# taithenguyen/ppls

Measured on AMD Instinct MI355X. Metric: accepted subintervals/sec + FP64 F-evals/sec at 1/2/4/8 MI355X, EPSILON=1e-10, higher is better.
Workload: dtype f64

## Files before the change

ppls_amd/csrc/aq_device.h:

```cpp
#pragma once
#include <hip/hip_runtime.h>
#include <stdint.h>

#include <type_traits>

#include "aquad.h"
#include "aq_libm.h"

#pragma clang fp contract(off)

namespace aq {

enum : unsigned { ERRB_TIMEOUT = 1, ERRB_OVERFLOW = 2, ERRB_DEPTH = 4 };

__device__ __forceinline__ unsigned cu_slot() {
    const unsigned hw = __builtin_amdgcn_s_getreg((31 << 11) | 4);
    const unsigned xcc = __builtin_amdgcn_s_getreg((3 << 11) | 20);
    const unsigned cu = (hw >> 8) & 15u, sh = (hw >> 12) & 1u, se = (hw >> 13) & 7u;
    return ((xcc & 7u) << 8) | (((se << 1) | sh) << 4) | cu;
}

__device__ __forceinline__ double wave_sum(double v) {
#pragma unroll
    for (int o = 32; o > 0; o >>= 1) v += __shfl_xor(v, o, 64);
// ... 121 lines not shown
            s[k].refine = fabs(s[k].area2 - lr2e[k]) > eps2;
            if constexpr (step_has_diff<S>) s[k].diff = s[k].area2 - lr2e[k];
        } else {
            const double lrarea = lr2e[k] / 2;
            const double larea = (fl[k] + fmid[k]) * wl[k] / 2;
            const double rarea = (fmid[k] + fr[k]) * wr[k] / 2;
            s[k].area2 = larea + rarea;
            s[k].refine = fabs((larea + rarea) - lrarea) > eps2;
            if constexpr (step_has_diff<S>) s[k].diff = (larea + rarea) - lrarea;
        }
    }
}

struct Step2c {
    double fmid, l2, r2, area2;
    bool refine;
};
template <int FID>
__device__ __forceinline__ void pair_step_carry(double ha, double hb, double fa, double fm, double fb, double lr0,
                                                double lr1, double eps2, const ExpEntry* __restrict__ tab,
                                                Step2c (&s)[2], double& m, double& hm, const ExpConsts& kk,
                                                int range_hint, unsigned long long out_mask) {
    static_assert(doubled_areas<FID>(), "carried areas are doubled areas");
    m = ha + hb;
    hm = 0.5 * m;
    const double mid[2] = {ha + hm, hm + hb};
    const double fl[2] = {fa, fm}, fr[2] = {fm, fb}, lr[2] = {lr0, lr1};
    double wl[2], wr[2];
    wl[0] = __fma_rn(ha, -2.0, mid[0]);
    wl[1] = mid[1] - m;
    wr[0] = m - mid[0];
    wr[1] = __fma_rn(hb, 2.0, -mid[1]);
#pragma unroll
    for (int k = 0; k < 2; ++k) asm volatile("" : "+v"(wl[k]), "+v"(wr[k]));
    double fmid[2];
    integrand_k<FID, 2, (f_scale<FID>() != 1.0)>(mid, fmid, tab, kk, range_hint, out_mask);
#pragma unroll
    for (int k = 0; k < 2; ++k) {
        s[k].fmid = fmid[k];
        s[k].l2 = (fl[k] + fmid[k]) * wl[k];
        s[k].r2 = (fmid[k] + fr[k]) * wr[k];
        s[k].area2 = s[k].l2 + s[k].r2;
        s[k].refine = fabs(s[k].area2 - lr[k]) > eps2;
    }
}

__host__ __device__ __forceinline__ void two_sum(double a, double b, double& s, double& e) {
    s = a + b;
    const double bb = s - a;
    e = (a - (s - bb)) + (b - bb);
}
__host__ __device__ __forceinline__ void dd_add(double& hi, double& lo, double v) {
    double s, e;
    two_sum(hi, v, s, e);
    hi = s;
    lo += e;
}
__host__ __device__ __forceinline__ void dd_add_dd(double& hi, double& lo, double h2, double l2) {
    double s, e;
    two_sum(hi, h2, s, e);
    e += lo + l2;
    two_sum(s, e, hi, lo);
}
__device__ __forceinline__ void masked_add(double& acc, double v, unsigned long long mask) {
    unsigned long long saved;
    asm("s_and_saveexec_b64 %1, %3\n\t"
        "v_add_f64 %0, %0, %2\n\t"
        "s_mov_b64 exec, %1"
        : "+v"(acc), "=&s"(saved)
        : "v"(v), "s"(mask)
        : "scc");
}

__device__ __forceinline__ void masked_max(unsigned& m, unsigned v, unsigned long long mask) {
    unsigned long long saved;
    asm("s_and_saveexec_b64 %1, %3\n\t"
        "v_max_u32 %0, %0, %2\n\t"
        "s_mov_b64 exec, %1"
        : "+v"(m), "=&s"(saved)
        : "v"(v), "s"(mask)
        : "scc");
}

__device__ __forceinline__ void masked_acc3(double& hi, double a0, unsigned long long l0m, double a1,
                                            unsigned long long l1m, unsigned& m, unsigned v, unsigned long long am) {
    unsigned long long saved;
    asm("s_mov_b64 %1, exec\n\t"
        "s_mov_b64 exec, %5\n\t"
        "v_add_f64 %0, %0, %3\n\t"
        "s_mov_b64 exec, %6\n\t"
        "v_add_f64 %0, %0, %4\n\t"
        "s_mov_b64 exec, %7\n\t"
        "v_max_u32_sdwa %2, %2, %8 dst_sel:DWORD dst_unused:UNUSED_PAD src0_sel:DWORD src1_sel:BYTE_0\n\t"
        "s_mov_b64 exec, %1"
        : "+v"(hi), "=&s"(saved), "+v"(m)
        : "v"(a0), "v"(a1), "s"(l0m), "s"(l1m), "s"(am), "v"(v));
}

__device__ __forceinline__ void masked_err4(double& sg, double& ab, double d0, unsigned long long l0m, double d1,
                                            unsigned long long l1m) {
    unsigned long long saved;
    asm("s_mov_b64 %2, exec\n\t"
        "s_mov_b64 exec, %5\n\t"
        "v_add_f64 %0, %0, %3\n\t"
        "v_add_f64 %1, %1, |%3|\n\t"
        "s_mov_b64 exec, %6\n\t"
        "v_add_f64 %0, %0, %4\n\t"
        "v_add_f64 %1, %1, |%4|\n\t"
        "s_mov_b64 exec, %2"
        : "+v"(sg), "+v"(ab), "=&s"(saved)
        : "v"(d0), "v"(d1), "s"(l0m), "s"(l1m));
}

__device__ __forceinline__ void wave_sum_dd(double& hi, double& lo) {
#pragma unroll
    for (int o = 32; o > 0; o >>= 1) {
        const double h2 = __shfl_xor(hi, o, 64), l2 = __shfl_xor(lo, o, 64);
        dd_add_dd(hi, lo, h2, l2);
    }
}

enum : int { DPP_XOR1 = 0xB1, DPP_XOR2 = 0x4E, DPP_HALF_MIRROR = 0x141, DPP_MIRROR = 0x140 };
template <int CTRL>
__device__ __forceinline__ unsigned dpp_u(unsigned v) {
    return (unsigned)__builtin_amdgcn_update_dpp(0, (int)v, CTRL, 0xF, 0xF, false);
}
template <int CTRL>
__device__ __forceinline__ double dpp_d(double v) {
    const unsigned long long b = (unsigned long long)__double_as_longlong(v);
    const unsigned lo = dpp_u<CTRL>((unsigned)b), hi = dpp_u<CTRL>((unsigned)(b >> 32));
    return __longlong_as_double((long long)(((unsigned long long)hi << 32) | lo));
}
__device__ __forceinline__ double readlane_d(double v, int l) {
    const unsigned long long b = (unsigned long long)__double_as_longlong(v);
    const unsigned lo = __builtin_amdgcn_readlane((unsigned)b, l), hi = __builtin_amdgcn_readlane((unsigned)(b >> 32), l);
    return __longlong_as_double((long long)(((unsigned long long)hi << 32) | lo));
}
template <typename Op>
__device__ __forceinline__ unsigned wave_reduce_u(unsigned v, Op op) {
    v = op(v, dpp_u<DPP_XOR1>(v));
    v = op(v, dpp_u<DPP_XOR2>(v));
    v = op(v, dpp_u<DPP_HALF_MIRROR>(v));
    v = op(v, dpp_u<DPP_MIRROR>(v));
    return op(op(__builtin_amdgcn_readlane(v, 0), __builtin_amdgcn_readlane(v, 16)),
              op(__builtin_amdgcn_readlane(v, 32), __builtin_amdgcn_readlane(v, 48)));
}
__device__ __forceinline__ unsigned wave_add_full(unsigned v) {
    return wave_reduce_u(v, [](unsigned x, unsigned y) { return x + y; });
}
__device__ __forceinline__ unsigned wave_max_full(unsigned v) {
    return wave_reduce_u(v, [](unsigned x, unsigned y) { return x > y ? x : y; });
}
__device__ __forceinline__ unsigned wave_or_full(unsigned v) {
    return wave_reduce_u(v, [](unsigned x, unsigned y) { return x | y; });
}
__device__ __forceinline__ double wave_sum_d_full(double v) {
    v += dpp_d<DPP_XOR1>(v);
    v += dpp_d<DPP_XOR2>(v);
    v += dpp_d<DPP_HALF_MIRROR>(v);
    v += dpp_d<DPP_MIRROR>(v);
    return (readlane_d(v, 0) + readlane_d(v, 16)) + (readlane_d(v, 32) + readlane_d(v, 48));
}
__device__ __forceinline__ void row_sum_dd(double& hi, double& lo) {
    double h2 = dpp_d<DPP_XOR1>(hi), l2 = dpp_d<DPP_XOR1>(lo);
    dd_add_dd(hi, lo, h2, l2);
    h2 = dpp_d<DPP_XOR2>(hi); l2 = dpp_d<DPP_XOR2>(lo);
    dd_add_dd(hi, lo, h2, l2);
    h2 = dpp_d<DPP_HALF_MIRROR>(hi); l2 = dpp_d<DPP_HALF_MIRROR>(lo);
    dd_add_dd(hi, lo, h2, l2);
    h2 = dpp_d<DPP_MIRROR>(hi); l2 = dpp_d<DPP_MIRROR>(lo);
    dd_add_dd(hi, lo, h2, l2);
}
__device__ __forceinline__ void wave_sum_dd_full(double& hi, double& lo) {
    double h2 = dpp_d<DPP_XOR1>(hi), l2 = dpp_d<DPP_XOR1>(lo);
    dd_add_dd(hi, lo, h2, l2);
    h2 = dpp_d<DPP_XOR2>(hi); l2 = dpp_d<DPP_XOR2>(lo);
    dd_add_dd(hi, lo, h2, l2);
    h2 = dpp_d<DPP_HALF_MIRROR>(hi); l2 = dpp_d<DPP_HALF_MIRROR>(lo);
    dd_add_dd(hi, lo, h2, l2);
    h2 = dpp_d<DPP_MIRROR>(hi); l2 = dpp_d<DPP_MIRROR>(lo);
    dd_add_dd(hi, lo, h2, l2);
    double h0 = readlane_d(hi, 0), l0 = readlane_d(lo, 0), h1 = readlane_d(hi, 16), l1 = readlane_d(lo, 16);
    double h3 = readlane_d(hi, 32), l3 = readlane_d(lo, 32);
    const double h4 = readlane_d(hi, 48), l4 = readlane_d(lo, 48);
    dd_add_dd(h0, l0, h1, l1);
    dd_add_dd(h3, l3, h4, l4);
    dd_add_dd(h0, l0, h3, l3);
    hi = h0;
    lo = l0;
}

__device__ __forceinline__ unsigned uni(unsigned v) { return __builtin_amdgcn_readfirstlane(v); }
__device__ __forceinline__ int uni(int v) { return __builtin_amdgcn_readfirstlane(v); }
__device__ __forceinline__ unsigned long long uni(unsigned long long v) {
    return ((unsigned long long)__builtin_amdgcn_readfirstlane((unsigned)(v >> 32)) << 32) |
// ... 41 lines not shown
```

ppls_amd/csrc/aq_stream.h:

```cpp
#pragma once
#include "aq_device.h"
#include "aq_shape.h"
#include "aq_xsum.h"

namespace aq {

typedef double f64x2 __attribute__((ext_vector_type(2)));

constexpr int PCAP = 128;
constexpr int DT_STRIDE = 2;
constexpr int LREC = NW * WCAP + PCAP;
constexpr int POOL0 = NW * WCAP;
constexpr int CH = PCAP;
struct DtField {
    unsigned* p;
    __device__ __forceinline__ unsigned& operator[](unsigned j) const { return p[DT_STRIDE * j]; }
    __device__ __forceinline__ DtField operator+(unsigned o) const { return DtField{p + DT_STRIDE * o}; }
};
#ifndef AQ_JOB_RUN_MAX
#define AQ_JOB_RUN_MAX 16
#endif
constexpr int JOB_RUN_MAX = AQ_JOB_RUN_MAX;
#ifndef AQ_GSS_DIV
#define AQ_GSS_DIV 2
// ... 239 lines not shown
    unsigned exited;
    unsigned long long tasks;
};

struct LdsPairs {
    double* a;
    double* b;
    double* fa;
    double* fm;
    double* fb;
    DtField dt;
};

__device__ __forceinline__ void wave_lock(int* lock, unsigned lane, unsigned long long& spins) {
    if (lane == 0) {
        int expect = 0;
        while (!__hip_atomic_compare_exchange_strong(lock, &expect, 1, __ATOMIC_ACQUIRE, __ATOMIC_RELAXED,
                                                     __HIP_MEMORY_SCOPE_WORKGROUP)) {
            expect = 0;
            ++spins;
            __builtin_amdgcn_s_sleep(1);
        }
    }
    __builtin_amdgcn_wave_barrier();
    __builtin_amdgcn_fence(__ATOMIC_ACQUIRE, "workgroup");
}

__device__ __forceinline__ void wave_unlock(int* lock, unsigned lane) {
    __builtin_amdgcn_fence(__ATOMIC_RELEASE, "workgroup");
    __builtin_amdgcn_wave_barrier();
    if (lane == 0) __hip_atomic_store(lock, 0, __ATOMIC_RELEASE, __HIP_MEMORY_SCOPE_WORKGROUP);
    __builtin_amdgcn_wave_barrier();
}

__device__ __forceinline__ void copy_pair(const LdsPairs& R, unsigned i, unsigned j) {
    const double a = R.a[i], b = R.b[i], fa = R.fa[i], fm = R.fm[i], fb = R.fb[i];
    const unsigned dt = R.dt[i];
    R.a[j] = a; R.b[j] = b; R.fa[j] = fa; R.fm[j] = fm; R.fb[j] = fb; R.dt[j] = dt;
}

template <typename SrcIdx>
__device__ __forceinline__ void publish_chunk(const StreamParams& P, const LdsPairs& R, unsigned slot, unsigned k,
                                              SrcIdx src, unsigned lane) {
    Chunk* __restrict__ c = P.chunks + slot;
    for (unsigned i = lane; i < k; i += 64) {
        const unsigned j = src(i);
        st_wt(&c->a[i], R.a[j]); st_wt(&c->b[i], R.b[j]);
        st_wt(&c->fa[i], R.fa[j]); st_wt(&c->fm[i], R.fm[j]); st_wt(&c->fb[i], R.fb[j]);
        st_wt(&c->dt[i], R.dt[j]);
    }
    if (lane == 0) st_wt(&c->count, k);
    asm volatile("s_waitcnt vmcnt(0)" ::: "memory");
    if (lane == 0) st_wt(&P.ready[(size_t)slot * READY_STRIDE], P.epoch);
}

struct Acc {
    double hi, lo;
    unsigned tasks, leaves, maxd;
    unsigned ut, ul;
    unsigned maxdt;
    double r = 0.0;
};

template <bool ERR>
struct ErrAcc {};
template <>
struct ErrAcc<true> {
    double sg = 0.0, ab = 0.0;
};

template <int FID, bool PCU, bool ERR = false>
__device__ __forceinline__ void flush_acc(const StreamParams& P, Acc& a, int tag, unsigned lane, WgState& S,
                                          unsigned long long* pc, double2* wdd, int wdd_stride, long long* xsa,
                                          long long* xsb, ErrAcc<ERR>& ea, double2* werr) {
    dd_add(a.hi, a.lo, a.r);
    a.r = 0.0;
    if (uni(a.ut) != 0u || __ballot(a.tasks != 0u) != 0ull) {
        double hi = area_scale<FID>() * a.hi, lo = area_scale<FID>() * a.lo;
#if AQ_FLUSHX == 1
        const unsigned t = a.ut + 1u, l = a.ul, m = 1u;
#elif AQ_FLUSHX == 3
        const unsigned mdt = wave_max_full(a.maxdt);
        const unsigned t = wave_add_full(a.tasks) + a.ut, l = wave_add_full(a.leaves) + a.ul,
                       m = max(wave_max_full(a.maxd), mdt ? (mdt & 255u) + 1u : 0u);
#elif AQ_FLUSHX == 4
        wave_sum_dd_full(hi, lo);
        const unsigned t = a.ut + 1u, l = a.ul, m = 1u;
#else
        if (PCU || !FLUSH_LDS) wave_sum_dd_full(hi, lo);
        const unsigned mdt = wave_max_full(a.maxdt);
        const unsigned t = wave_add_full(a.tasks) + a.ut, l = wave_add_full(a.leaves) + a.ul,
                       m = max(wave_max_full(a.maxd), mdt ? (mdt & 255u) + 1u : 0u);
#endif
        if constexpr (!PCU && FLUSH_LDS) {
            if (t) {
                xsa[lane] = 0ll;
                if (lane < 4u) xsb[lane] = 0ll;
                auto add_digits = [&](double v) {
                    XDigits g;
                    if (!xs_digits(v, g)) return;
#pragma unroll
                    for (int k = 0; k < 3; ++k) {
                        const int i = g.i + k;
                        if (g.d[k]) atomicAdd(reinterpret_cast<unsigned long long*>(i < 64 ? &xsa[i] : &xsb[i - 64]),
                                              (unsigned long long)g.d[k]);
                    }
                };
                add_digits(area_scale<FID>() * a.hi);
                add_digits(area_scale<FID>() * a.lo);
                const long long v0 = xsa[lane], v1 = lane < 4u ? xsb[lane] : 0ll;
                Ctl& c = P.ctls[P.first_slot + tag];
                if (v0) atomicAdd(reinterpret_cast<unsigned long long*>(&c.area.limb[lane]), (unsigned long long)v0);
                if (v1) atomicAdd(reinterpret_cast<unsigned long long*>(&c.area.limb[64 + lane]), (unsigned long long)v1);
                const unsigned long long nz0 = __ballot(v0 != 0ll), nz1 = __ballot(v1 != 0ll);
                if ((nz0 | nz1) && lane == 0u) {
                    const int lo_nz = nz0 ? __builtin_ctzll(nz0) : 64 + __builtin_ctzll(nz1);
                    const int hi_nz = nz1 ? 64 + (63 - __builtin_clzll(nz1)) : 63 - __builtin_clzll(nz0);
                    atomicMax(&c.sums.win_lo_not, xs_win_lo(lo_nz));
                    atomicMax(&c.sums.win_hi, (unsigned)(hi_nz + 1));
                }
            }
        }
        if constexpr (ERR) {
            const double eab = area_scale<FID>() * wave_sum_d_full(ea.ab), esg = area_scale<FID>() * wave_sum_d_full(ea.sg);
            if (lane == 0 && t) {
                if constexpr (PCU) {
                    double2& w = werr[tag * wdd_stride];
                    w = make_double2(w.x + eab, w.y + esg);
                } else {
                    double* e = P.err + 2 * (size_t)(P.first_slot + tag);
                    unsafeAtomicAdd(e, eab);
                    unsafeAtomicAdd(e + 1, esg);
                }
            }
        }
        if (AQ_FLUSHX != 2 && lane == 0 && t) {
            atomicAdd(&S.tasks, (unsigned long long)t);
            if constexpr (PCU) {
                atomicAdd(&pc[tag], (unsigned long long)t);
                atomicAdd(&pc[PCU_ROW + tag], (unsigned long long)l);
                atomicMax(&pc[2 * PCU_ROW + tag], (unsigned long long)m);
                double2& w = wdd[tag * wdd_stride];
                double wh = w.x, wl = w.y;
                dd_add_dd(wh, wl, hi, lo);
                w = make_double2(wh, wl);
            } else {
                Ctl& c = P.ctls[P.first_slot + tag];
                atomicAdd(&c.sums.tasks, (unsigned long long)t);
                atomicAdd(&c.sums.leaves, (unsigned long long)l);
                atomicMax(&c.sums.levels, m);
                if constexpr (!FLUSH_LDS) {
                    const int i0 = xs_atomic_add(c.area.limb, hi);
                    const int i1 = xs_atomic_add(c.area.limb, lo);
                    xs_window_add(c.sums, i0, i1);
                }
            }
        }
    }
    a.hi = a.lo = 0.0;
    a.tasks = a.leaves = a.maxd = 0;
    a.ut = a.ul = 0;
    a.maxdt = 0;
    if constexpr (ERR) ea.sg = ea.ab = 0.0;
    __builtin_amdgcn_wave_barrier();
}

typedef unsigned u32x4 __attribute__((ext_vector_type(4)));
__device__ __forceinline__ double2 sload_bounds(const double2* base, int p) {
    const unsigned long long a64 = (unsigned long long)(base + p);
    const unsigned long long addr = ((unsigned long long)(unsigned)__builtin_amdgcn_readfirstlane((int)(a64 >> 32)) << 32) |
                                    (unsigned)__builtin_amdgcn_readfirstlane((int)(unsigned)a64);
    u32x4 r;
    asm volatile("s_load_dwordx4 %0, %1, 0x0\n\ts_waitcnt lgkmcnt(0)" : "=s"(r) : "s"(addr) : "memory");
    return make_double2(__hiloint2double((int)r.y, (int)r.x), __hiloint2double((int)r.w, (int)r.z));
}

typedef unsigned u32x2 __attribute__((ext_vector_type(2)));
template <int FID>
__device__ __forceinline__ void sload_theta(Theta<FID>& th, const double* base, int p) {
    if constexpr (FID == F_PARAM) {
        constexpr int NP = param::nparams;
        const unsigned long long a64 = (unsigned long long)(base + (size_t)p * NP);
        const unsigned long long addr = ((unsigned long long)(unsigned)__builtin_amdgcn_readfirstlane((int)(a64 >> 32)) << 32) |
                                        (unsigned)__builtin_amdgcn_readfirstlane((int)(unsigned)a64);
#pragma unroll
        for (int i = 0; i < NP; i += 2) {
            const unsigned long long ai = addr + 8ull * (unsigned)i;
            if (i + 1 < NP) {
                u32x4 r;
                asm volatile("s_load_dwordx4 %0, %1, 0x0\n\ts_waitcnt lgkmcnt(0)" : "=s"(r) : "s"(ai) : "memory");
                th.v[i] = __hiloint2double((int)r.y, (int)r.x);
                th.v[i + 1 < NP ? i + 1 : i] = __hiloint2double((int)r.w, (int)r.z);
            } else {
                u32x2 r;
                asm volatile("s_load_dwordx2 %0, %1, 0x0\n\ts_waitcnt lgkmcnt(0)" : "=s"(r) : "s"(ai) : "memory");
                th.v[i] = __hiloint2double((int)r.y, (int)r.x);
            }
        }
    }
}

static_assert(LREC * 8 == 50 * 512, "the pair moves assume 50 x 512 B per field");
__device__ __forceinline__ void lds_pop6_masked(unsigned long long m, unsigned addr, unsigned addr2, double& a,
                                                double& b, double& fa, double& fm, double& fb, double& dw) {
    unsigned long long saved;
    asm volatile(
        "s_mov_b64 %6, exec\n\t"
        "s_mov_b64 exec, %7\n\t"
        "ds_read_b64 %0, %8\n\t"
        "ds_read_b64 %1, %8 offset:25600\n\t"
        "ds_read_b64 %2, %8 offset:51200\n\t"
        "ds_read_b64 %3, %9\n\t"
        "ds_read_b64 %4, %9 offset:25600\n\t"
        "ds_read_b64 %5, %9 offset:51200\n\t"
        "s_mov_b64 exec, %6\n\t"
        "s_waitcnt lgkmcnt(0)"
        : "+v"(a), "+v"(b), "+v"(fa), "+v"(fm), "+v"(fb), "+v"(dw), "=&s"(saved)
        : "s"(m), "v"(addr), "v"(addr2)
        : "memory");
}
__device__ __forceinline__ void lds_push6_masked(unsigned long long m, unsigned addr, double x0, double x1, double x2,
                                                 double x3, double x4, double x5) {
    unsigned long long saved;
    asm volatile(
        "s_mov_b64 %0, exec\n\t"
        "s_mov_b64 exec, %1\n\t"
        "ds_write2st64_b64 %2, %3, %4 offset1:50\n\t"
        "ds_write2st64_b64 %2, %5, %6 offset0:100 offset1:150\n\t"
        "ds_write2st64_b64 %2, %7, %8 offset0:200 offset1:250\n\t"
        "s_mov_b64 exec, %0"
        : "=&s"(saved)
        : "s"(m), "v"(addr), "v"(x0), "v"(x1), "v"(x2), "v"(x3), "v"(x4), "v"(x5)
        : "memory");
}
struct PairRegs {
    f64x2 ab, ff, fd;
};
__device__ __forceinline__ void lds_issue6(unsigned addr, PairRegs& r) {
    asm volatile(
        "ds_read2st64_b64 %0, %3 offset1:50\n\t"
        "ds_read2st64_b64 %1, %3 offset0:100 offset1:150\n\t"
        "ds_read2st64_b64 %2, %3 offset0:200 offset1:250"
        : "=&v"(r.ab), "=&v"(r.ff), "=&v"(r.fd)
        : "v"(addr)
        : "memory");
}
__device__ __forceinline__ void lds_wait6(PairRegs& r) {
    asm volatile("s_waitcnt lgkmcnt(0)" : "+v"(r.ab), "+v"(r.ff), "+v"(r.fd) : : "memory");
}
__device__ __forceinline__ void lds_store6(unsigned addr, const PairRegs& r) {
    asm volatile(
        "ds_write2st64_b64 %0, %1, %2 offset1:50\n\t"
        "ds_write2st64_b64 %0, %3, %4 offset0:100 offset1:150\n\t"
        "ds_write2st64_b64 %0, %5, %6 offset0:200 offset1:250"
        :
        : "v"(addr), "v"(r.ab.x), "v"(r.ab.y), "v"(r.ff.x), "v"(r.ff.y), "v"(r.fd.x), "v"(r.fd.y)
        : "memory");
}
__device__ __forceinline__ PairRegs chunk_load(const CellarChunk* ch, unsigned lane) {
    return PairRegs{ch->ab[lane], ch->ff[lane], ch->fd[lane]};
}
__device__ __forceinline__ void chunk_store(CellarChunk* ch, unsigned lane, const PairRegs& r) {
    ch->ab[lane] = r.ab;
    ch->ff[lane] = r.ff;
    ch->fd[lane] = r.fd;
}
__device__ __forceinline__ unsigned ring_addr(unsigned ring8, unsigned i, unsigned vmask) {
    return ((i << 3) & vmask) | ring8;
}
__device__ __forceinline__ unsigned ring_slot(unsigned i) { return i % (unsigned)WCAP; }
__device__ __forceinline__ unsigned ring_wrap(unsigned v) {
    if constexpr ((WCAP & (WCAP - 1)) == 0) return v & (unsigned)(WCAP - 1);
    else return min(v, v - (unsigned)WCAP);
}

#if AQ_STAMPS
__device__ unsigned long long g_aq_stamps[MAXG * NW * ST_STRIDE];
#endif

template <int FID, bool HIST, bool DIAG, bool PCU, int NWT = NW, bool HEAPS = false, bool ERR = false>
__global__ __launch_bounds__(NWT * 64) void k_stream(StreamParams P) {
    static_assert(!ERR || (!HIST && !DIAG), "ERR launches keep no histograms and no diagnostics");
    constexpr int PTT = NWT * 64;
    static_assert(NWT >= 4 && NWT <= NW && NWT % 4 == 0, "whole waves per SIMD, within the LDS rings");
    static_assert(NWT <= 16, "the exit's area sum runs over one DPP row of lanes (PCU_AREA)");
    constexpr bool WIDE = AQ_WIDE_TAB && FID == F_COSH4 && !PCU;
    constexpr int TAB_FRONT = WIDE ? 256 * 16 / 8 : 0;
    __shared__ double s_lds[TAB_FRONT + 6 * LREC];
    double* const s_pr = s_lds + TAB_FRONT;
    __shared__ ExpEntry tab_own[WIDE ? 1 : ftab_entries<FID>()];
    ExpEntry* const tab = WIDE ? reinterpret_cast<ExpEntry*>(s_lds) : tab_own;
    const DtField s_dt{reinterpret_cast<unsigned*>(s_pr + 5 * LREC)};
    double* const s_a = s_pr;
    double* const s_b = s_pr + LREC;
    double* const s_fa = s_pr + 2 * LREC;
    double* const s_fm = s_pr + 3 * LREC;
    double* const s_fb = s_pr + 4 * LREC;
    __shared__ WgState S;
    __shared__ unsigned long long s_pc[PCU ? 3 * PCU_ROW : 1];
    __shared__ double2 s_wdd[PCU ? PCU_ROW * NWT : 1];
    __shared__ double2 s_werr[PCU && ERR ? PCU_ROW * NWT : 1];
    __shared__ unsigned long long s_dg[DIAG ? DIAG_WORDS : 1];

    const unsigned tid = threadIdx.x;
    const unsigned lane = lane_id();
    const unsigned wid = __builtin_amdgcn_readfirstlane(tid >> 6);
    const unsigned bid = __builtin_amdgcn_readfirstlane(blockIdx.x);
    QCtl* __restrict__ qc = P.q;
    const LdsPairs R{s_a, s_b, s_fa, s_fm, s_fb, s_dt};
    const unsigned pr_base = (unsigned)(uintptr_t)s_pr;
    const unsigned long long t_entry = (DIAG || AQ_STAMPS) ? rtc() : 0ull;
    unsigned long long stp[ST_N] = {};
    auto stamp = [&](int k) {
        if constexpr (AQ_STAMPS && !DIAG) { if (!stp[k]) stp[k] = rtc(); }
    };
    stp[ST_ENTRY] = t_entry;
    if constexpr (AQ_STAMPS && !DIAG) {
        asm volatile("" :: "s"(P.eps), "s"(P.shares), "s"(P.nprob), "s"(P.kbounds[0].x));
        stamp(ST_KARG);
    }
    ExpPair tv{};
    if (FID != F_SIN_RECIP && tid < (WIDE ? 256u : 128u)) tv = reinterpret_cast<const ExpPair*>(kExpTabBits)[tid & 127u];
    static_assert(FID != F_SIN_RECIP || AQ_SINCOS_TAB_N <= PTT, "one sin-table entry per thread");
    double sv = 0.0;
    if (FID == F_SIN_RECIP && tid < (unsigned)AQ_SINCOS_TAB_N) sv = kSinCosTab[tid];
    stamp(ST_PRE);
    if (bid == 0)
        for (unsigned i = tid; i < (unsigned)(sizeof(QCtl) / 4); i += PTT) reinterpret_cast<unsigned*>(P.q_next)[i] = 0u;
    if (tid == 0) {
        S.lock = 0; S.pbot = 0; S.ptop = 0; S.idle = 0; S.phase = 0; S.busy_token = 1;
        S.exited = 0; S.tasks = 0;
    }
    if (PCU && tid < 3u * PCU_ROW) s_pc[tid] = 0ull;
    if (PCU)
        for (unsigned i = tid; i < (unsigned)(PCU_ROW * NWT); i += PTT) s_wdd[i] = make_double2(0.0, 0.0);
    if constexpr (PCU && ERR)
        for (unsigned i = tid; i < (unsigned)(PCU_ROW * NWT); i += PTT) s_werr[i] = make_double2(0.0, 0.0);
    if (DIAG) {
        for (unsigned i = tid; i < DIAG_WORDS; i += PTT) s_dg[i] = (i == DG_T_FIRST_LEAD) ? ~0ull : 0ull;
    }
// ... 857 lines not shown
                    if (lane == 0) spilled += k;
                    if constexpr (DIAG) {
                        if (lane == 0) {
                            atomicAdd(&s_dg[DG_CHUNKS_OUT], 1ull);
                            atomicAdd(&s_dg[DG_RECORDS_OUT], (unsigned long long)k);
                        }
                    }
                    __builtin_amdgcn_wave_barrier();
                    continue;
                }
            }
        }

        if ((poll_ctr % give_rounds) == 0 && size >= give_min &&
            uni(__hip_atomic_load(&S.idle, __ATOMIC_RELAXED, __HIP_MEMORY_SCOPE_WORKGROUP)) > 0 &&
            uni(__hip_atomic_load(&S.ptop, __ATOMIC_RELAXED, __HIP_MEMORY_SCOPE_WORKGROUP)) ==
                uni(__hip_atomic_load(&S.pbot, __ATOMIC_RELAXED, __HIP_MEMORY_SCOPE_WORKGROUP))) {
            const unsigned k = size / 2u;
            wave_lock(&S.lock, lane, lock_spins);
            const unsigned pt = uni(S.ptop);
            const bool fits = (pt - S.pbot) + k <= (unsigned)PCAP;
            if (fits) {
                for (unsigned i = lane; i < k; i += 64)
                    copy_pair(R, base + ring_slot(bot + i), POOL0 + ((pt + i) & (PCAP - 1)));
                if (lane == 0) S.ptop = pt + k;
            }
            wave_unlock(&S.lock, lane);
            if constexpr (DIAG) { if (lane == 0) atomicAdd(&s_dg[DG_GIVE], (unsigned long long)(fits ? k : 0u)); }
            if (fits) {
                bot += k;
                __builtin_amdgcn_wave_barrier();
                continue;
            }
        }
        if (ctop > 0 && pf_n == 0 && size <= (unsigned)PF_ISSUE) {
            pf_n = 64u;
            ctop -= pf_n;
            pf = chunk_load(&cel->c[ctop / 64u], lane);
            __builtin_amdgcn_wave_barrier();
        }

        unsigned long long cb0 = 0;
        if constexpr (AQ_STAMPS && !DIAG) cb0 = clk();
        unsigned b_top = uni(top), b_size = uni(size), b_poll = uni(poll_ctr);
        unsigned b_n = 0;
        unsigned long long b_dv = 0;
        unsigned b_bot = uni(bot), b_ctop = uni(ctop), b_pf = uni(pf_n);
        bool b_mixed = uni(mixed);
        unsigned b_S = b_size, b_S0 = b_size;
        unsigned long long b_am = 0;
        double ca = 0.0, cb = 0.0, cfa = 0.0, cfm = 0.0, cfb = 0.0, cdw = 0.0;
        unsigned b_lo1, b_span;
        auto window = [&]() {
            b_lo1 = (b_pf != 0u ? (unsigned)PF_BELOW : (b_ctop > 0u ? (unsigned)PF_ISSUE : 0u)) + 1u;
            b_span = (unsigned)(WCAP - 64) + 1u - b_lo1;
        };
        window();
        constexpr bool prio_by_load = PCU && FID == F_SIN_RECIP;
        const bool b_heavy = prio_by_load && b_S >= HEAVY_S;
        const unsigned b_max = give_rounds - b_poll % give_rounds;
        unsigned b_rem = b_max;
        __builtin_amdgcn_s_waitcnt(0xC07F);
        bool b_go;
        for (;;) {
        for (;;) {
            unsigned long long c0 = 0, c1 = 0;
            if constexpr (DIAG) c0 = clk();
            if constexpr (prio_by_load) {
                if (b_heavy) asm volatile("s_setprio 3");
                else asm volatile("s_setprio 1");
            }
            const unsigned long long need = ~b_am;
            const unsigned k = min((unsigned)__popcll(need), b_top - b_bot);
            const unsigned jr = mbcnt(need);
            const unsigned long long fmsk = __ballot(jr < k) & need;
            b_top -= k;
            const unsigned paddr = ring_addr(ring8, ring_slot(b_top) + jr, ring_vmask);
            lds_pop6_masked(fmsk, paddr, paddr + 3u * 50u * 512u, ca, cb, cfa, cfm, cfb, cdw);
            const unsigned long long am = b_am | fmsk;
            const unsigned na = (unsigned)__popcll(am);
            const double pa = ca, pb = cb, pfa = cfa, pfm = cfm, pfb = cfb;
            const unsigned long long dtw = (unsigned long long)__double_as_longlong(cdw);
            const unsigned dt = (unsigned)dtw;
            using StepT = typename std::conditional<ERR, Step2e, Step2>::type;
            StepT st[2];
            unsigned long long nospan = 0ull;
            if constexpr (FID == F_COSH4) nospan = __ballot((int)dt >= 0);
            double pm, hm;
            pair_step_halves<FID, WIDE ? 255u : 127u, StepT>(pa, pb, pfa, pfm, pfb, eps2, tab, st, pm, hm, kk,
                                                              FID == F_COSH4 ? 2 : -1, nospan & am, th);
            if constexpr (prio_by_load) { if (!b_heavy) asm volatile("s_setprio 0"); }
            const unsigned long long r0m = __ballot(st[0].refine), r1m = __ballot(st[1].refine);
            unsigned long long okm = am;
            if constexpr (!burst_cap) {
                const unsigned long long dm = __ballot((dt & 255u) < (unsigned)(max_depth - 1));
                okm = am & dm;
                const unsigned long long atcap = am & ~dm;
                if (__builtin_expect(atcap != 0ull, 0)) b_dv |= atcap & (r0m | r1m);
            }
            const unsigned long long l0m = am & ~r0m, l1m = am & ~r1m;
            b_n += na;
            const unsigned long long mask0 = okm & r0m, mask1 = okm & r1m;
            const unsigned cdt = dt + 1u;
            const unsigned long long cdtw = ((dtw >> 32) << 32) | (unsigned long long)cdt;
            masked_acc3(acc.r, st[0].area2, l0m, st[1].area2, l1m, acc.maxdt, burst_cap ? cdt : dt,
                        burst_cap ? (mask0 | mask1) : am);
            if constexpr (ERR) masked_err4(eacc.sg, eacc.ab, st[0].diff, l0m, st[1].diff, l1m);
            if constexpr (DIAG) {
                const int rtag = (int)dt_tag(dt);
                b_mixed |= (__ballot(rtag != tag) & am) != 0ull;
            }
            if (HIST) {
                const unsigned d = dt & 255u;
                if (__builtin_amdgcn_inverse_ballot_w64(am)) {
                    atomicAdd(&P.ctls[P.first_slot + tag].hist[d], 2ull);
                    const unsigned nl = ((l0m >> lane) & 1u) + ((l1m >> lane) & 1u);
                    if (nl) atomicAdd(&P.ctls[P.first_slot + tag].hist[AQ_MAX_LEVELS + d], (unsigned long long)nl);
                }
            }
            if constexpr (DIAG) c1 = clk();
            lds_push6_masked(mask1, ring_addr(ring8, ring_slot(b_top) + mbcnt(mask1), ring_vmask), hm, pb, pfm,
                             st[1].fmid, pfb, __longlong_as_double((long long)cdtw));
            b_top += (unsigned)__popcll(mask1);
            cb = hm;
            cfb = pfm;
            cfm = st[0].fmid;
            cdw = __longlong_as_double((long long)cdtw);
            b_am = mask0;
            if constexpr (DIAG) {
                if (lane == 0) {
                    const unsigned long long c2 = clk();
                    atomicAdd(&s_dg[DG_ROUNDS], 1ull);
                    atomicAdd(&s_dg[DG_ACTIVE_LANES], (unsigned long long)na);
                    atomicAdd(&s_dg[DG_C_ROUND], c2 - c0);
                    atomicAdd(&s_dg[DG_C_EVAL], c1 - c0);
                    atomicMax(&s_dg[DG_MAX_RING], (unsigned long long)b_S);
                    atomicMax(&s_dg[DG_T_LAST_ROUND], rtc());
                    atomicAdd(&s_dg[DG_ACTIVE_TASKS], 2ull * na);
                }
            }
            b_S = (b_top - b_bot) + (unsigned)__popcll(mask0);
            --b_rem;
            unsigned span_r = b_rem != 0u ? b_span : 0u;
            asm("" : "+s"(span_r));
            b_go = b_S - b_lo1 < span_r;
            __builtin_amdgcn_wave_barrier();
            if (!b_go) break;
        }
            unsigned b_re = b_rem;
            asm volatile("" : "+s"(b_re));
            const unsigned sz = b_S;
            if (b_re != 0u && sz != 0u) {
                if (sz > (unsigned)(WCAP - 64)) {
                    if (b_ctop + (unsigned)SPILL <= (unsigned)CCAP) {
                        if (b_pf) {
                            b_ctop += b_pf;
                            b_pf = 0;
                        }
                        spill_to_cellar(b_bot, b_ctop);
                        b_ctop += (unsigned)SPILL;
                        b_bot += (unsigned)SPILL;
                        b_S -= (unsigned)SPILL;
                        b_S0 -= (unsigned)SPILL;
                        b_go = true;
                    }
                } else if (b_pf) {
                    if (b_bot < 64u) {
                        b_bot += (unsigned)WCAP;
                        b_top += (unsigned)WCAP;
                    }
                    b_bot -= b_pf;
                    if (lane < b_pf) lds_store6(ring_addr(ring8, ring_slot(b_bot) + lane, ring_vmask), pf);
                    if constexpr (DIAG) { if (lane == 0) atomicAdd(&s_dg[DG_PREFETCH], (unsigned long long)b_pf); }
                    b_S += b_pf;
                    b_S0 += b_pf;
                    b_pf = 0;
                    b_go = true;
                } else if (b_ctop > 0u) {
                    b_pf = 64u;
                    b_ctop -= 64u;
                    pf = chunk_load(&cel->c[b_ctop / 64u], lane);
                    b_go = true;
                }
                if (b_go) window();
            }
            __builtin_amdgcn_wave_barrier();
            if (!b_go) break;
        }
        if constexpr (prio_by_load) asm volatile("s_setprio 0");
        lds_push6_masked(b_am, ring_addr(ring8, ring_slot(b_top) + mbcnt(b_am), ring_vmask), ca, cb, cfa, cfm, cfb,
                         cdw);
        b_top += (unsigned)__popcll(b_am);
        bot = b_bot;
        ctop = b_ctop;
        pf_n = b_pf;
        b_poll += (b_max - b_rem) - 1u;
        top = b_top;
        poll_ctr = b_poll;
        acc.ut += 2u * b_n;
        acc.ul += b_n - ((b_top - b_bot) - b_S0);
        dd_add(acc.hi, acc.lo, acc.r);
        acc.r = 0.0;
        if (b_dv) err |= ERRB_DEPTH;
        if constexpr (burst_cap) {
            if (__builtin_expect(__ballot((acc.maxdt & 255u) >= (unsigned)max_depth) != 0ull, 0)) {
                err |= ERRB_DEPTH;
                top = bot;
                ctop = 0;
                pf_n = 0;
            }
        }
        mixed = b_mixed;
        if constexpr (AQ_STAMPS && !DIAG) {
            stp[ST_CB] += clk() - cb0;
            stp[ST_NB] += 1ull;
            stp[ST_NR] += (unsigned long long)(b_max - b_rem);
        }
        __builtin_amdgcn_wave_barrier();
    }

    if constexpr (DIAG) { if (lane == 0) atomicMax(&s_dg[DG_T_BROKE], rtc()); }
    stamp(ST_BROKE);
    flush_acc<FID, PCU, ERR>(P, acc, tag, lane, S, s_pc, s_wdd + wid, NWT, xs_a, xs_b, eacc, s_werr + wid);
    if constexpr (DIAG) { if (lane == 0) atomicMax(&s_dg[DG_T_FLUSHED], rtc()); }
    stamp(ST_FLUSHED);
    if (mixed) err |= ERRB_OVERFLOW;
    const unsigned werr = wave_or_full(err);
    unsigned last_u = 0;
    if (lane == 0) {
        if (werr) {
            for (int p = 0; p < P.nprob; ++p)
                atomicOr(&P.ctls[P.first_slot + p].sums.error, werr);
        }
        if (spilled) atomicAdd(&P.ctls[P.first_slot].sums.spilled, spilled);
        if constexpr (DIAG) {
            atomicAdd(&s_dg[DG_LOCK_SPINS], lock_spins);
            atomicAdd(&s_dg[DG_SPILL_RECORDS], spilled);
            atomicAdd(&s_dg[DG_C_LOOP], clk() - cl0);
        }
        __builtin_amdgcn_fence(__ATOMIC_RELEASE, "workgroup");
        const bool last = atomicAdd(&S.exited, 1u) == (unsigned)NWT - 1u;
        __builtin_amdgcn_fence(__ATOMIC_ACQUIRE, "workgroup");
        last_u = last ? 1u : 0u;
        if (last) {
            const unsigned long long wt = __hip_atomic_load(&S.tasks, __ATOMIC_RELAXED, __HIP_MEMORY_SCOPE_WORKGROUP);
            if (wt && !AQ_X_NOCUACC) __hip_atomic_fetch_add(&P.cu_acc[cu_slot()], wt, __ATOMIC_RELAXED, __HIP_MEMORY_SCOPE_AGENT);
        }
        if constexpr (DIAG) { if (last) atomicMax(&s_dg[DG_T_FOLD], rtc()); }
        if (PCU && last) {
            const unsigned cu = cu_slot();
            for (int p = 0; p < P.nprob; ++p) {
                const unsigned long long t = __hip_atomic_load(&s_pc[p], __ATOMIC_RELAXED, __HIP_MEMORY_SCOPE_WORKGROUP);
                const unsigned long long l = __hip_atomic_load(&s_pc[PCU_ROW + p], __ATOMIC_RELAXED, __HIP_MEMORY_SCOPE_WORKGROUP);
                const unsigned m = (unsigned)__hip_atomic_load(&s_pc[2 * PCU_ROW + p], __ATOMIC_RELAXED, __HIP_MEMORY_SCOPE_WORKGROUP);
                unsigned long long* wp = P.parts + 2 * ((size_t)p * gridDim.x + bid);
                wp[0] = pack_cu(t, cu);
                wp[1] = (l << 8) | (unsigned long long)(m & 255u);
                if (bid == 0) {
                    SlotSums& sm = P.ctls[P.first_slot + p].sums;
                    sm.pcu = 1u;
                    sm.win_lo_not = xs_win_lo(0);
                    sm.win_hi = (unsigned)XS_LIMBS;
                }
            }
        }
        if (!PCU && last && (P.adaptive & 2)) {
            const unsigned long long wt = __hip_atomic_load(&S.tasks, __ATOMIC_RELAXED, __HIP_MEMORY_SCOPE_WORKGROUP);
            __hip_atomic_fetch_add(&P.hint->tasks, wt, __ATOMIC_RELAXED, __HIP_MEMORY_SCOPE_AGENT);
            const unsigned g = __hip_atomic_fetch_add(&P.hint->exits, 1u, __ATOMIC_ACQ_REL, __HIP_MEMORY_SCOPE_AGENT);
            if (g == gridDim.x - 1u) {
                const unsigned long long tot = __hip_atomic_load(&P.hint->tasks, __ATOMIC_ACQUIRE, __HIP_MEMORY_SCOPE_AGENT);
                const unsigned long long per = tot / (unsigned long long)P.nprob;
                unsigned long long sh = (per + TASKS_PER_JOB / 2) / TASKS_PER_JOB;
                sh = sh < 1ull ? 1ull : (sh > (unsigned long long)W ? (unsigned long long)W : sh);
                __hip_atomic_store(&P.hint->shares_next, (unsigned)sh, __ATOMIC_RELAXED, __HIP_MEMORY_SCOPE_AGENT);
                if constexpr (HEAPS) __hip_atomic_store(&P.hint->per_next, per, __ATOMIC_RELAXED, __HIP_MEMORY_SCOPE_AGENT);
                __hip_atomic_store(&P.hint->tasks, 0ull, __ATOMIC_RELAXED, __HIP_MEMORY_SCOPE_AGENT);
                __hip_atomic_store(&P.hint->exits, 0u, __ATOMIC_RELAXED, __HIP_MEMORY_SCOPE_AGENT);
            }
        }
    }
    if constexpr (PCU && !AQ_X_NOFOLD) {
        if (uni(__shfl(last_u, 0, 64))) {
            for (int p = 0; p < P.nprob; ++p) {
                double hi = 0.0, lo = 0.0;
                if (lane < (unsigned)NWT) {
                    const double2 w = s_wdd[p * NWT + (int)lane];
                    hi = w.x;
                    lo = w.y;
                }
                row_sum_dd(hi, lo);
                if (lane == 0) {
// ... 48 lines not shown
```

Baseline: 300.9 billion.

## Fuse refine test, accumulation and ring push into one exec-masked asm block

Replaces the separate ballots for refine masks, the masked accumulate and error-sum helpers, and the separate LDS ring push with one inline-asm sequence. It uses v_cmpx to derive the leaf masks directly from |diff| against eps and writes the refined children to the ring under the resulting exec mask. This aims to cut scalar ballot/exec shuffling and instruction count in the hot round loop. It always uses the Step2e step type so diff is available, records the child depth in maxdt with adjusted flush arithmetic, and replaces the burst-cap depth abort with a scan of ring depth entries so the abort fires only when a task actually reaches max depth. This adds register pressure and an LDS scan on the rare depth path.

After: 302.3 billion (median of 6 runs). No clear change (+0.5%).

```diff
diff --git a/ppls_amd/csrc/aq_device.h b/ppls_amd/csrc/aq_device.h
--- a/ppls_amd/csrc/aq_device.h
+++ b/ppls_amd/csrc/aq_device.h
@@ -227,35 +227,63 @@
         : "scc");
 }
 
-__device__ __forceinline__ void masked_acc3(double& hi, double a0, unsigned long long l0m, double a1,
-                                            unsigned long long l1m, unsigned& m, unsigned v, unsigned long long am) {
+#define AQ_TAIL_OPEN                                                                                          \
+    "s_mov_b64 %[sv], exec\n\t"                                                                               \
+    "s_mov_b64 exec, %[am]\n\t"                                                                               \
+    "v_max_u32_sdwa %[m], %[m], %[dt] dst_sel:DWORD dst_unused:UNUSED_PAD src0_sel:DWORD src1_sel:BYTE_0\n\t" \
+    "v_cmpx_ngt_f64_e64 %[l0], |%[d0]|, %[eps]\n\t"                                                           \
+    "v_add_f64 %[hi], %[hi], %[a0]\n\t"
+#define AQ_TAIL_MID                                 \
+    "s_mov_b64 exec, %[am]\n\t"                     \
+    "v_cmpx_ngt_f64_e64 %[l1], |%[d1]|, %[eps]\n\t" \
+    "v_add_f64 %[hi], %[hi], %[a1]\n\t"
+#define AQ_TAIL_PUSH                                                    \
+    "s_andn2_b64 exec, %[okm], exec\n\t"                                \
+    "v_mbcnt_lo_u32_b32 %[ad], exec_lo, 0\n\t"                          \
+    "v_mbcnt_hi_u32_b32 %[ad], exec_hi, %[ad]\n\t"                      \
+    "v_add_lshl_u32 %[ad], %[ad], %[slot], 3\n\t"                       \
+    "v_and_or_b32 %[ad], %[ad], %[vm], %[r8]\n\t"                       \
+    "ds_write2st64_b64 %[ad], %[x0], %[x1] offset1:50\n\t"              \
+    "ds_write2st64_b64 %[ad], %[x2], %[x3] offset0:100 offset1:150\n\t" \
+    "ds_write2st64_b64 %[ad], %[x4], %[x5] offset0:200 offset1:250\n\t" \
+    "s_mov_b64 exec, %[sv]"
+#define AQ_TAIL_INPUTS                                                                                              \
+    [dt] "v"(dt), [a0] "v"(a0), [d0] "v"(d0), [a1] "v"(a1), [d1] "v"(d1), [eps] "v"(eps2), [am] "s"(am),            \
+        [okm] "s"(okm), [slot] "s"(slot), [vm] "v"(vmask), [r8] "s"(ring8), [x0] "v"(x0), [x1] "v"(x1), [x2] "v"(x2), \
+        [x3] "v"(x3), [x4] "v"(x4), [x5] "v"(x5)
+__device__ __forceinline__ void round_tail(double& hi, unsigned& m, unsigned dt, double a0, double d0, double a1,
+                                           double d1, double eps2, unsigned long long am, unsigned long long okm,
+                                           unsigned long long& l0m, unsigned long long& l1m, unsigned slot,
+                                           unsigned vmask, unsigned ring8, double x0, double x1, double x2, double x3,
+                                           double x4, double x5) {
     unsigned long long saved;
-    asm("s_mov_b64 %1, exec\n\t"
-        "s_mov_b64 exec, %5\n\t"
-        "v_add_f64 %0, %0, %3\n\t"
-        "s_mov_b64 exec, %6\n\t"
-        "v_add_f64 %0, %0, %4\n\t"
-        "s_mov_b64 exec, %7\n\t"
-        "v_max_u32_sdwa %2, %2, %8 dst_sel:DWORD dst_unused:UNUSED_PAD src0_sel:DWORD src1_sel:BYTE_0\n\t"
-        "s_mov_b64 exec, %1"
-        : "+v"(hi), "=&s"(saved), "+v"(m)
-        : "v"(a0), "v"(a1), "s"(l0m), "s"(l1m), "s"(am), "v"(v));
-}
-
-__device__ __forceinline__ void masked_err4(double& sg, double& ab, double d0, unsigned long long l0m, double d1,
-                                            unsigned long long l1m) {
+    unsigned addr;
+    asm volatile(AQ_TAIL_OPEN AQ_TAIL_MID AQ_TAIL_PUSH
+                 : [hi] "+v"(hi), [m] "+v"(m), [sv] "=&s"(saved), [l0] "=&s"(l0m), [l1] "=&s"(l1m), [ad] "=&v"(addr)
+                 : AQ_TAIL_INPUTS
+                 : "memory", "scc");
+}
+__device__ __forceinline__ void round_tail_err(double& hi, unsigned& m, unsigned dt, double a0, double d0, double a1,
+                                               double d1, double eps2, unsigned long long am, unsigned long long okm,
+                                               unsigned long long& l0m, unsigned long long& l1m, unsigned slot,
+                                               unsigned vmask, unsigned ring8, double x0, double x1, double x2,
+                                               double x3, double x4, double x5, double& sg, double& ab) {
     unsigned long long saved;
-    asm("s_mov_b64 %2, exec\n\t"
-        "s_mov_b64 exec, %5\n\t"
-        "v_add_f64 %0, %0, %3\n\t"
-        "v_add_f64 %1, %1, |%3|\n\t"
-        "s_mov_b64 exec, %6\n\t"
-        "v_add_f64 %0, %0, %4\n\t"
-        "v_add_f64 %1, %1, |%4|\n\t"
-        "s_mov_b64 exec, %2"
-        : "+v"(sg), "+v"(ab), "=&s"(saved)
-        : "v"(d0), "v"(d1), "s"(l0m), "s"(l1m));
-}
+    unsigned addr;
+    asm volatile(AQ_TAIL_OPEN
+                 "v_add_f64 %[sg], %[sg], %[d0]\n\t"
+                 "v_add_f64 %[ab], %[ab], |%[d0]|\n\t" AQ_TAIL_MID
+                 "v_add_f64 %[sg], %[sg], %[d1]\n\t"
+                 "v_add_f64 %[ab], %[ab], |%[d1]|\n\t" AQ_TAIL_PUSH
+                 : [hi] "+v"(hi), [m] "+v"(m), [sv] "=&s"(saved), [l0] "=&s"(l0m), [l1] "=&s"(l1m), [ad] "=&v"(addr),
+                   [sg] "+v"(sg), [ab] "+v"(ab)
+                 : AQ_TAIL_INPUTS
+                 : "memory", "scc");
+}
+#undef AQ_TAIL_OPEN
+#undef AQ_TAIL_MID
+#undef AQ_TAIL_PUSH
+#undef AQ_TAIL_INPUTS
 
 __device__ __forceinline__ void wave_sum_dd(double& hi, double& lo) {
 #pragma unroll
diff --git a/ppls_amd/csrc/aq_stream.h b/ppls_amd/csrc/aq_stream.h
--- a/ppls_amd/csrc/aq_stream.h
+++ b/ppls_amd/csrc/aq_stream.h
@@ -345,7 +345,7 @@
 #elif AQ_FLUSHX == 3
         const unsigned mdt = wave_max_full(a.maxdt);
         const unsigned t = wave_add_full(a.tasks) + a.ut, l = wave_add_full(a.leaves) + a.ul,
-                       m = max(wave_max_full(a.maxd), mdt ? (mdt & 255u) + 1u : 0u);
+                       m = max(wave_max_full(a.maxd), mdt & 255u);
 #elif AQ_FLUSHX == 4
         wave_sum_dd_full(hi, lo);
         const unsigned t = a.ut + 1u, l = a.ul, m = 1u;
@@ -353,7 +353,7 @@
         if (PCU || !FLUSH_LDS) wave_sum_dd_full(hi, lo);
         const unsigned mdt = wave_max_full(a.maxdt);
         const unsigned t = wave_add_full(a.tasks) + a.ut, l = wave_add_full(a.leaves) + a.ul,
-                       m = max(wave_max_full(a.maxd), mdt ? (mdt & 255u) + 1u : 0u);
+                       m = max(wave_max_full(a.maxd), mdt & 255u);
 #endif
         if constexpr (!PCU && FLUSH_LDS) {
             if (t) {
@@ -519,6 +519,11 @@
         :
         : "v"(addr), "v"(r.ab.x), "v"(r.ab.y), "v"(r.ff.x), "v"(r.ff.y), "v"(r.fd.x), "v"(r.fd.y)
         : "memory");
+}
+__device__ __forceinline__ unsigned lds_dt_lo(unsigned addr) {
+    unsigned v;
+    asm volatile("ds_read_b32 %0, %1\n\ts_waitcnt lgkmcnt(0)" : "=v"(v) : "v"(addr + 250u * 512u) : "memory");
+    return v;
 }
 __device__ __forceinline__ PairRegs chunk_load(const CellarChunk* ch, unsigned lane) {
     return PairRegs{ch->ab[lane], ch->ff[lane], ch->fd[lane]};
@@ -1542,7 +1547,7 @@
             const double pa = ca, pb = cb, pfa = cfa, pfm = cfm, pfb = cfb;
             const unsigned long long dtw = (unsigned long long)__double_as_longlong(cdw);
             const unsigned dt = (unsigned)dtw;
-            using StepT = typename std::conditional<ERR, Step2e, Step2>::type;
+            using StepT = Step2e;
             StepT st[2];
             unsigned long long nospan = 0ull;
             if constexpr (FID == F_COSH4) nospan = __ballot((int)dt >= 0);
@@ -1550,22 +1555,29 @@
             pair_step_halves<FID, WIDE ? 255u : 127u, StepT>(pa, pb, pfa, pfm, pfb, eps2, tab, st, pm, hm, kk,
                                                               FID == F_COSH4 ? 2 : -1, nospan & am, th);
             if constexpr (prio_by_load) { if (!b_heavy) asm volatile("s_setprio 0"); }
-            const unsigned long long r0m = __ballot(st[0].refine), r1m = __ballot(st[1].refine);
-            unsigned long long okm = am;
+            unsigned long long okm = am, atcap = 0ull;
             if constexpr (!burst_cap) {
                 const unsigned long long dm = __ballot((dt & 255u) < (unsigned)(max_depth - 1));
                 okm = am & dm;
-                const unsigned long long atcap = am & ~dm;
-                if (__builtin_expect(atcap != 0ull, 0)) b_dv |= atcap & (r0m | r1m);
-            }
-            const unsigned long long l0m = am & ~r0m, l1m = am & ~r1m;
+                atcap = am & ~dm;
+            }
             b_n += na;
-            const unsigned long long mask0 = okm & r0m, mask1 = okm & r1m;
             const unsigned cdt = dt + 1u;
             const unsigned long long cdtw = ((dtw >> 32) << 32) | (unsigned long long)cdt;
-            masked_acc3(acc.r, st[0].area2, l0m, st[1].area2, l1m, acc.maxdt, burst_cap ? cdt : dt,
-                        burst_cap ? (mask0 | mask1) : am);
-            if constexpr (ERR) masked_err4(eacc.sg, eacc.ab, st[0].diff, l0m, st[1].diff, l1m);
+            if constexpr (DIAG) c1 = clk();
+            unsigned long long l0m, l1m;
+            if constexpr (ERR)
+                round_tail_err(acc.r, acc.maxdt, cdt, st[0].area2, st[0].diff, st[1].area2, st[1].diff, eps2, am, okm,
+                               l0m, l1m, ring_slot(b_top), ring_vmask, ring8, hm, pb, pfm, st[1].fmid, pfb,
+                               __longlong_as_double((long long)cdtw), eacc.sg, eacc.ab);
+            else
+                round_tail(acc.r, acc.maxdt, cdt, st[0].area2, st[0].diff, st[1].area2, st[1].diff, eps2, am, okm, l0m,
+                           l1m, ring_slot(b_top), ring_vmask, ring8, hm, pb, pfm, st[1].fmid, pfb,
+                           __longlong_as_double((long long)cdtw));
+            const unsigned long long mask0 = okm & ~l0m, mask1 = okm & ~l1m;
+            if constexpr (!burst_cap) {
+                if (__builtin_expect(atcap != 0ull, 0)) b_dv |= atcap & ~(l0m & l1m);
+            }
             if constexpr (DIAG) {
                 const int rtag = (int)dt_tag(dt);
                 b_mixed |= (__ballot(rtag != tag) & am) != 0ull;
@@ -1578,9 +1590,6 @@
                     if (nl) atomicAdd(&P.ctls[P.first_slot + tag].hist[AQ_MAX_LEVELS + d], (unsigned long long)nl);
                 }
             }
-            if constexpr (DIAG) c1 = clk();
-            lds_push6_masked(mask1, ring_addr(ring8, ring_slot(b_top) + mbcnt(mask1), ring_vmask), hm, pb, pfm,
-                             st[1].fmid, pfb, __longlong_as_double((long long)cdtw));
             b_top += (unsigned)__popcll(mask1);
             cb = hm;
             cfb = pfm;
@@ -1664,10 +1673,16 @@
         if (b_dv) err |= ERRB_DEPTH;
         if constexpr (burst_cap) {
             if (__builtin_expect(__ballot((acc.maxdt & 255u) >= (unsigned)max_depth) != 0ull, 0)) {
-                err |= ERRB_DEPTH;
-                top = bot;
-                ctop = 0;
-                pf_n = 0;
+                bool deep = (acc.maxdt & 255u) > (unsigned)max_depth;
+                for (unsigned i = lane; i < top - bot; i += 64u)
+                    deep |= (lds_dt_lo(ring_addr(ring8, ring_slot(bot + i), ring_vmask)) & 255u) >= (unsigned)max_depth;
+                if (__ballot(deep) != 0ull) {
+                    err |= ERRB_DEPTH;
+                    top = bot;
+                    ctop = 0;
+                    pf_n = 0;
+                }
+                __builtin_amdgcn_wave_barrier();
             }
         }
         mixed = b_mixed;
```
